# SUNGBEOMCHOI/Rubiks-Cube-Solver

Hardware: NVIDIA B200
Metric: cube transitions/sec (higher is better)
Workload: dtype u8

## Files before the change

rubiks_cube_solver_b200/csrc/build.py:

```python
import os
import subprocess
import sys

HERE = os.path.dirname(os.path.abspath(__file__))
PKG = os.path.dirname(HERE)
LIB = os.path.join(PKG, "libcube_b200.so")
SOURCES = ["scramble.cu", "prefix.cu", "walk.cu", "sched.cu", "expand.cu", "leaf.cu", "decode.cu", "adi.cu", "seeds.cu", "mcts.cu", "pipeline.cu", "envhost.cu", "peer.cu", "abi.cu"]
HEADERS = ["cube_common.cuh", "cube_threads.cuh", "cube_bulk.cuh", "cube_sched.cuh", "cube_tables.cuh", "cube_kernels.h", os.path.join("..", "..", "include", "cube_b200.h")]
NVCC_FLAGS = ["-O3", "-std=c++17", "-gencode", "arch=compute_100a,code=sm_100a", "-lineinfo",
              "-Xcompiler", "-fPIC", "-shared"]


def nvcc():
    for cand in (os.environ.get("NVCC"), "/usr/local/cuda/bin/nvcc", "nvcc"):
        if cand and (os.path.isabs(cand) and os.path.exists(cand) or not os.path.isabs(cand)):
            return cand
    return "nvcc"


def stale():
    if not os.path.exists(LIB):
        return True
    t = os.path.getmtime(LIB)
    return any(os.path.getmtime(os.path.join(HERE, f)) > t
               for f in SOURCES + HEADERS if os.path.exists(os.path.join(HERE, f)))


def build(force=False, verbose=False):
    from concurrent.futures import ThreadPoolExecutor
    srcs = [s for s in SOURCES if os.path.exists(os.path.join(HERE, s))]
    if not force and not stale():
        return LIB
    objdir = os.path.join(HERE, "build")
    os.makedirs(objdir, exist_ok=True)
    hdr_t = max(os.path.getmtime(os.path.join(HERE, h)) for h in HEADERS + ["build.py"] if os.path.exists(os.path.join(HERE, h)))
    compile_flags = [f for f in NVCC_FLAGS if f != "-shared"] + (["-Xptxas", "-v"] if verbose else [])

    def compile_one(src):
        obj = os.path.join(objdir, src[:-3] + ".o")
        if not force and os.path.exists(obj) and os.path.getmtime(obj) > max(hdr_t, os.path.getmtime(os.path.join(HERE, src))):
            return obj
        tmp_o = obj + ".tmp%d" % os.getpid()
        try:
            subprocess.check_call([nvcc()] + compile_flags + ["-c", "-o", tmp_o, src], cwd=HERE)
            os.replace(tmp_o, obj)
        finally:
            if os.path.exists(tmp_o):
                os.remove(tmp_o)
        return obj

    with ThreadPoolExecutor(max_workers=min(len(srcs), os.cpu_count() or 4)) as pool:
        objs = list(pool.map(compile_one, srcs))
    tmp = LIB + ".tmp%d" % os.getpid()
    try:
        subprocess.check_call([nvcc()] + NVCC_FLAGS + ["-o", tmp] + objs, cwd=HERE)
        os.replace(tmp, LIB)
    finally:
        if os.path.exists(tmp):
            os.remove(tmp)
    return LIB

# ... 4 lines not shown
```

rubiks_cube_solver_b200/csrc/cube_kernels.h:

```cpp
#pragma once
#include <cstdint>
#include <cuda_runtime.h>
#include "../../include/cube_b200.h"

namespace cube {

int launch_scramble(int size, const uint8_t* moves, long long n, int depth, uint8_t* states_out,
                    uint8_t* solved, float* reward, unsigned long long* counters, cudaStream_t stream,
                    const uint8_t* last = nullptr);

int launch_prefixes(int size, const uint8_t* moves, long long n, int depth, uint8_t* states_out, uint8_t* solved,
                    unsigned long long* counters, cudaStream_t stream);
int prefix_max_depth(int size);

int launch_walk(int size, const uint8_t* states_in, const uint8_t* moves, long long n, int depth,
                uint8_t* states_out, uint8_t* solved, float* reward, unsigned long long* counters,
                cudaStream_t stream);

int launch_solved(int size, const uint8_t* states, long long n, uint8_t* solved, float* reward,
                  unsigned long long* counters, cudaStream_t stream);

int launch_expand(int size, const uint8_t* states, long long n, uint8_t* children, void* child_onehot,
                  void* parent_onehot, int dtype, uint8_t* solved, float* reward,
                  unsigned long long* counters, cudaStream_t stream, int encoding = CUBE_ENCODING_REFERENCE);

int launch_expand_codes(int size, const uint8_t* states, long long n, uint8_t* children, uint8_t* child_codes,
                        uint8_t* parent_codes, void* parent_onehot, int dtype, uint8_t* solved, float* reward,
                        unsigned long long* counters, cudaStream_t stream, int encoding = CUBE_ENCODING_REFERENCE);

int launch_validate(int size, const uint8_t* actions, long long count, unsigned long long* counters,
                    cudaStream_t stream);

long long launch_leaf2(const uint8_t* states, long long n, uint8_t* children, void* parent_onehot, int dtype,
                       uint8_t* solved, float* reward, unsigned long long* counters, cudaStream_t stream, int* rc);

int launch_seeded_moves(int size, const uint32_t* seeds, long long n, int depth, uint8_t* moves,
                        unsigned long long* counters, cudaStream_t stream);

int launch_adi_targets(int size, const float* child_values, const uint8_t* child_solved, const float* parent_values,
                       const int* scramble_count, const double* weight, int table_len, long long n,
                       float* target_value, int* target_policy, double* error, cudaStream_t stream);

long long launch_leaf2_children(const uint8_t* states, long long n, uint8_t* children, void* child_onehot,
                                void* parent_onehot, int dtype, uint8_t* solved, float* reward,
                                unsigned long long* counters, cudaStream_t stream, int* rc);

int launch_mcts_traverse(int size, const cube_mcts_tree_t& t, float cpuct, int virtual_loss, cudaStream_t stream);
int launch_mcts_update(int size, const cube_mcts_tree_t& t, const uint8_t* leaf_key, const uint8_t* child_key_new,
                       const uint8_t* child_done_new, const float* value, const float* policy, float value_min,
                       int sim_index, int8_t* actions_out, int* n_actions, int* n_sims, int* n_active, cudaStream_t stream);

int launch_decode2(const void* onehot, int dtype, long long n, uint8_t* out, cudaStream_t stream);
int launch_decode3_exact(const void* onehot, int dtype, long long n, uint8_t* out, cudaStream_t stream);

size_t peer_buffer_bytes(int cap);
int launch_peer_allreduce_i64(int world, int rank, const uint64_t* peer_bufs, long long* values, int n, int cap,
                              unsigned epoch, cudaStream_t stream);

int sm_count();
int device_slot();
int persistent_ctas();

}
```

rubiks_cube_solver_b200/csrc/cube_sched.cuh:

```cuda
#pragma once
#include <cstdint>
#include <cuda_runtime.h>

namespace sched {

constexpr int kClaimChunk = 2;
constexpr int kRanges = 8;
constexpr int kTailDiv = 4;
constexpr int kSlots = 1024;
constexpr int kExhausted = 0x7fffff00;

struct Slot { unsigned next[kRanges][32]; unsigned ctas_done; unsigned tail_div; unsigned pad[30]; };

Slot* claim_slot();
int tail_div();

struct WarpTiles {
    Slot* slot;
    int n_tiles, total_warps, tail0;
    int next_static;
    int r, visited;
    int cur, end;
    int chunk;
    unsigned pending;

    __device__ __forceinline__ int lo(int range) const
    {
        return tail0 + (int)((long long)range * (n_tiles - tail0) / kRanges);
    }
    __device__ __forceinline__ void claim_ahead(int lane)
    {
        if (lane == 0) pending = atomicAdd(&slot->next[r][0], (unsigned)chunk);
    }

    __device__ __forceinline__ void init(Slot* s, int n, int warps_per_cta, int warp, int lane, int tail_div,
                                         int claim_chunk = kClaimChunk)
    {
        slot = s; n_tiles = n; total_warps = (int)gridDim.x * warps_per_cta; chunk = claim_chunk;
        const int gid = (int)blockIdx.x * warps_per_cta + warp;
        tail0 = tail_div > 0 ? n - n / tail_div : n;
        next_static = gid;
        r = gid % kRanges; visited = 0; cur = end = 0; pending = 0;
        if (next_static >= tail0) claim_ahead(lane);
    }

    __device__ __forceinline__ int pop(int lane)
    {
        if (next_static < tail0) {
            const int t = next_static;
            next_static += total_warps;
            if (next_static >= tail0) claim_ahead(lane);
            return t;
        }
        while (cur >= end) {
            if (visited >= kRanges) return kExhausted;
            const unsigned got = __shfl_sync(0xffffffffu, pending, 0);
            const int hi = lo(r + 1);
            const long long base = (long long)lo(r) + got;
            if (base < hi) {
                cur = (int)base;
                end = cur + chunk < hi ? cur + chunk : hi;
            } else {
                bool left = false;
                if (lane < kRanges) left = lo(lane) + (long long)__ldcg(&slot->next[lane][0]) < lo(lane + 1);
                const unsigned open = __ballot_sync(0xffffffffu, left) & ((1u << kRanges) - 1u);
                if (open == 0) { visited = kRanges; return kExhausted; }
                const unsigned rot = (open >> (r + 1)) | (open << (kRanges - r - 1));
                r = (r + 1 + (__ffs(rot & ((1u << kRanges) - 1u)) - 1)) % kRanges;
            }
            claim_ahead(lane);
        }
        return cur++;
    }
};

__device__ __forceinline__ void release(Slot* slot)
{
    if (threadIdx.x == 0) {
        __threadfence();
        if (atomicAdd(&slot->ctas_done, 1u) == gridDim.x - 1) {
            for (int i = 0; i < kRanges; ++i) slot->next[i][0] = 0;
            slot->ctas_done = 0;
            __threadfence();
        }
    }
}

}
```

rubiks_cube_solver_b200/csrc/sched.cu:

```cuda
#include <atomic>
#include <cstdlib>
#include "cube_sched.cuh"

namespace sched {

__device__ Slot g_slots[kSlots];

Slot* claim_slot()
{
    static std::atomic<unsigned> seq{0};
    static Slot* base[64] = {};
    int dev = 0;
    if (cudaGetDevice(&dev) != cudaSuccess || dev < 0 || dev >= 64) return nullptr;
    Slot* b = base[dev];
    if (!b) {
        void* p = nullptr;
        if (cudaGetSymbolAddress(&p, g_slots) != cudaSuccess) return nullptr;
        b = base[dev] = static_cast<Slot*>(p);
    }
    return b + (seq.fetch_add(1, std::memory_order_relaxed) % kSlots);
}

int tail_div()
{
    static int v = -1;
    if (v < 0) {
        const char* e = getenv("CUBE_TAIL_DIV");
        v = e ? atoi(e) : kTailDiv;
        if (v < 0) v = kTailDiv;
    }
    return v;
}

}
```

rubiks_cube_solver_b200/csrc/scramble.cu:

```cuda
#include <atomic>
#include <cstdlib>
#include <cstring>
#include <cuda.h>
#include <cuda_runtime.h>
#include "cube_bulk.cuh"
#include "cube_kernels.h"
#include "cube_sched.cuh"
#include "cube_threads.cuh"

namespace {

#ifndef CUBE_SCRAMBLE_MIN_BLOCKS
#define CUBE_SCRAMBLE_MIN_BLOCKS 6
#endif
constexpr int kTile = 256;
constexpr int kMaxStagedDepth = 160;

__host__ __device__ constexpr int round16(int x) { return (x + 15) & ~15; }

template <int SIZE>
struct ScrambleSmem {
    using G = CubeGeom<SIZE>;
    static constexpr int kTable = 0;
    static constexpr int kCornerLut = kTable + G::MW * CUBE_MOVE_ROWS * 4;
// ... 83 lines not shown
        }
    } else {
        const long long byte0 = base * G::S;
        const int nbytes = cnt * G::S;
        for (int i = tid; i < nbytes; i += kTile) out[byte0 + i] = s_out[i];
    }
    if (tid < cnt) {
        const bool row_ok = s_flags[tid] != 0;
        if (solved) solved[base + tid] = row_ok ? 1 : 0;
        if (reward) reward[base + tid] = row_ok ? 1.0f : -1.0f;
    }
    if (full && tid == 0) bulk::wait_read_all();
}


constexpr int kMaxPairDepth = 320;
constexpr int kPairTableBytes = CUBE_PAIR_ROWS * 256;
template <int SIZE, int NS> struct PairCfg;
template <> struct PairCfg<3, 2> { static constexpr int kMaxWarps = 24; };
template <> struct PairCfg<2, 2> { static constexpr int kMaxWarps = 32; };
template <> struct PairCfg<2, 4> { static constexpr int kMaxWarps = 20; };
constexpr int kMinWarpsFour = 16;

template <int SIZE, int NS>
struct PairSmem {
    using G = CubeGeom<SIZE>;
    static constexpr int kPairTile = 32 * NS;
    static constexpr int kTable = 0;
    static constexpr int kCornerLut = kPairTableBytes + 256;
    static constexpr int kEdgeLut = kCornerLut + 256;
    static constexpr int kPerWarp = (kEdgeLut + (SIZE == 3 ? 1536 : 256) + 1023) / 1024 * 1024;
    static constexpr int kOutBytes = kPairTile * G::S;
    __host__ __device__ static constexpr int round1k(int x) { return (x + 1023) & ~1023; }
    __host__ __device__ static constexpr int move_stride(int depth, bool swz = false)
    {
        return swz ? round1k(kPairTile * depth) : kPairTile * depth + 16;
    }
    __host__ __device__ static constexpr int moves_at(bool swz = false) { return swz ? round1k(16 + kOutBytes) : 16 + kOutBytes; }
    __host__ __device__ static constexpr int per_warp(int depth, bool swz = false)
    {
        return moves_at(swz) + 2 * move_stride(depth, swz);
    }
    __host__ __device__ static constexpr int bytes(int depth, int warps, bool priv = false)
    {
        return kPerWarp + warps * per_warp(depth, priv) < 66048 ? 66048 : kPerWarp + warps * per_warp(depth, priv);
    }
};

template <int SIZE, int DEPTH, int NS, int MODE>
__global__ void __launch_bounds__(PairCfg<SIZE, NS>::kMaxWarps * 32, 1)
scramble_pairs_kernel(const uint8_t* __restrict__ moves, int n_tiles, int depth_rt, uint8_t* __restrict__ out,
                      uint8_t* __restrict__ solved, float* __restrict__ reward, unsigned long long* __restrict__ counters,
                      sched::Slot* slot, int tail_div, const __grid_constant__ CUtensorMap move_map,
                      const uint8_t* __restrict__ last)
{
    using L = PairSmem<SIZE, NS>;
    constexpr int kPairTile = L::kPairTile;
    extern __shared__ __align__(128) uint8_t smem_raw[];
    const int depth = DEPTH > 0 ? DEPTH : depth_rt;
    constexpr bool kPriv = DEPTH < 0;
    constexpr uint32_t kAlign = kPriv ? 1024u : 256u;
    const int tid = threadIdx.x, lane = tid & 31, warp = tid >> 5;
    const uint32_t window = bulk::smem_addr(smem_raw);
    uint8_t* smem = smem_raw + ((kAlign - (window & (kAlign - 1u))) & (kAlign - 1u));
    uint8_t* s_ptbl = smem + L::kTable;
    const PairTableShared tbl{bulk::smem_addr(s_ptbl)};
    uint32_t* s_clut = reinterpret_cast<uint32_t*>(smem + L::kCornerLut);
    uint32_t* s_elut = reinterpret_cast<uint32_t*>(smem + L::kEdgeLut);
    uint8_t* mine = smem + L::kPerWarp + warp * L::per_warp(depth, kPriv);
    uint64_t* s_bar = reinterpret_cast<uint64_t*>(mine);
    uint8_t* s_out = mine + 16;
    uint8_t* s_moves = mine + L::moves_at(kPriv);
    const int mstride = L::move_stride(depth, kPriv);
    const uint32_t move_bytes = (uint32_t)(kPairTile * depth);
    auto stage = [&](int t, int b) {
        if (bulk::elect_one()) {
            bulk::mbar_expect_tx(&s_bar[b], move_bytes);
            if (!kPriv) bulk::load(s_moves + b * mstride, moves + (long long)t * move_bytes, move_bytes, &s_bar[b]);
            else bulk::load_tile_2d(s_moves + b * mstride, &move_map, 0, t * (kPairTile * depth >> 7), &s_bar[b]);
        }
    };

    asm volatile("griddepcontrol.launch_dependents;");
    pair_table_fill<SIZE>(s_ptbl, tid, blockDim.x);
    if (tid < 32) s_clut[tid] = (SIZE == 3) ? kCornerColour3[tid] : kCornerColour2[tid];
    if (SIZE == 3) for (int i = tid; i < 12 * 32; i += blockDim.x) s_elut[i] = kEdgeColourSlot3[i];
    if (lane == 0) { bulk::mbar_init(&s_bar[0], 1); bulk::mbar_init(&s_bar[1], 1); }
    if (lane == 0 && depth > 0) {
        const int total = (int)gridDim.x * (int)(blockDim.x >> 5);
#pragma unroll
        for (int k = 0; k < 2; ++k) {
            const int t = (int)blockIdx.x * (int)(blockDim.x >> 5) + warp + k * total;
            if (t < n_tiles) bulk::prefetch_l2(moves + (long long)t * move_bytes, move_bytes);
        }
    }
    __syncthreads();
    asm volatile("griddepcontrol.wait;" ::: "memory");

    sched::WarpTiles tiles;
    tiles.init(slot, n_tiles, (int)(blockDim.x >> 5), warp, lane, tail_div);
    int tile = tiles.pop(lane);
    if (tile < n_tiles) stage(tile, 0);
    int rows[NS];
#pragma unroll
    for (int k = 0; k < NS; ++k) rows[k] = (SIZE == 3) ? 64 * (k >> 1) + 2 * lane + (k & 1) : lane + 32 * k;
    const uint32_t lanereg = pair_lanereg<SIZE>(lane, tbl), roff = pair_roff2(lane);
    const ColourLutShared lut{bulk::smem_addr(s_clut), bulk::smem_addr(s_elut)};
    unsigned n_solved = 0;
    const bool has_last = MODE == 2 || (MODE == 0 && last != nullptr);
    const bool has_solved = MODE != 0 || solved != nullptr, has_reward = MODE != 0 || reward != nullptr;
    for (int it = 0; tile < n_tiles; ++it) {
        const int buf = it & 1;
        const int next = tiles.pop(lane);
        if (next < n_tiles) stage(next, buf ^ 1);
        uint32_t last_w[NS];
        if (has_last) {
            if (SIZE == 3) {
#pragma unroll
                for (int h = 0; h < NS; h += 2) {
                    const uint32_t v = *reinterpret_cast<const uint16_t*>(last + (long long)tile * kPairTile + 32 * h + 2 * lane);
                    last_w[h] = v & 0xffu; last_w[h + 1] = v >> 8;
                }
            } else {
#pragma unroll
                for (int k = 0; k < NS; ++k) last_w[k] = last[(long long)tile * kPairTile + 32 * k + lane];
            }
        }
        bulk::mbar_wait(&s_bar[buf], (uint32_t)(it >> 1) & 1u);

        CubieState st[NS];
#pragma unroll
        for (int k = 0; k < NS; ++k) cubie_init(st[k]);
        if constexpr (kPriv) scramble_pairs_run_swizzled<SIZE, NS>(st, s_moves + buf * mstride, lane, depth, tbl, lanereg, roff);
        else scramble_pairs_run<SIZE, (DEPTH > 0 ? DEPTH : 0), NS>(st, rows, depth, s_moves + buf * mstride, tbl, lanereg, roff);
        if (has_last) {
#pragma unroll
            for (int k = 0; k < NS; ++k) scramble_pairs_last<SIZE>(st[k], last_w[k], tbl, lanereg, roff);
        }
        if (bulk::elect_one()) bulk::wait_read_all();
        __syncwarp();
        bool ok[NS];
#pragma unroll
        for (int k = 0; k < NS; ++k) {
            ok[k] = scramble_pairs_finish<SIZE>(st[k], rows[k], lut, s_out);
            n_solved += ok[k] ? 1u : 0u;
        }

        bulk::fence_smem_writes();
        __syncwarp();
        if (bulk::elect_one()) {
            bulk::store(out + (long long)tile * L::kOutBytes, s_out, (uint32_t)L::kOutBytes);
            bulk::commit();
        }
        if (SIZE == 3) {
#pragma unroll
            for (int h = 0; h < NS; h += 2) {
                const long long r0 = (long long)tile * kPairTile + 32 * h + 2 * lane;
                if (has_solved) *reinterpret_cast<uint16_t*>(solved + r0) = (uint16_t)((ok[h] ? 1u : 0u) | (ok[h + 1] ? 0x100u : 0u));
                if (has_reward) *reinterpret_cast<float2*>(reward + r0) = make_float2(ok[h] ? 1.0f : -1.0f, ok[h + 1] ? 1.0f : -1.0f);
            }
        } else {
#pragma unroll
            for (int k = 0; k < NS; ++k) {
                if (has_solved) solved[(long long)tile * kPairTile + 32 * k + lane] = ok[k] ? 1 : 0;
                if (has_reward) reward[(long long)tile * kPairTile + 32 * k + lane] = ok[k] ? 1.0f : -1.0f;
            }
        }
        tile = next;
    }
    n_solved = __reduce_add_sync(0xffffffffu, n_solved);
    if (lane == 0 && n_solved && counters) atomicAdd(&counters[0], (unsigned long long)n_solved);
    if (blockIdx.x == 0 && tid == 0 && counters) atomicAdd(&counters[1], (unsigned long long)n_tiles * kPairTile);
    __syncwarp();
    if (bulk::elect_one()) bulk::wait_read_all();
    __syncthreads();
    sched::release(slot);
}

constexpr int kSliceDefault = 112;
__host__ __device__ constexpr int slice_stride(int slice) { return ((slice + 32) / 16) % 2 ? slice + 32 : slice + 48; }

template <int SIZE>
struct SlicedSmem {
    using G = CubeGeom<SIZE>;
    static constexpr int kOutBytes = 64 * G::S;
    static constexpr int kMovesAt = 16 + kOutBytes;
    __host__ __device__ static constexpr int per_warp(int slice) { return kMovesAt + 2 * 64 * slice_stride(slice); }
    static constexpr int kFixed = PairSmem<SIZE, 2>::kPerWarp;
    __host__ __device__ static constexpr int bytes(int warps, int slice) { return kFixed + warps * per_warp(slice); }
};

template <int SIZE>
__global__ void __launch_bounds__(8 * 32, 1)
scramble_sliced_kernel(const uint8_t* __restrict__ moves, int n_tiles, int depth, uint8_t* __restrict__ out,
                       uint8_t* __restrict__ solved, float* __restrict__ reward, unsigned long long* __restrict__ counters,
                       const uint8_t* __restrict__ last, int kSlice)
{
    using L = SlicedSmem<SIZE>;
    using P = PairSmem<SIZE, 2>;
    extern __shared__ __align__(128) uint8_t smem_raw[];
    const int tid = threadIdx.x, lane = tid & 31, warp = tid >> 5, warps = (int)(blockDim.x >> 5);
    const uint32_t window = bulk::smem_addr(smem_raw);
    uint8_t* smem = smem_raw + ((256u - (window & 255u)) & 255u);
    uint8_t* s_ptbl = smem + P::kTable;
    const PairTableShared tbl{bulk::smem_addr(s_ptbl)};
    uint32_t* s_clut = reinterpret_cast<uint32_t*>(smem + P::kCornerLut);
    uint32_t* s_elut = reinterpret_cast<uint32_t*>(smem + P::kEdgeLut);
    const int kSliceStride = slice_stride(kSlice);
    uint8_t* mine = smem + L::kFixed + warp * L::per_warp(kSlice);
    uint64_t* s_bar = reinterpret_cast<uint64_t*>(mine);
    uint8_t* s_out = mine + 16;
    uint8_t* s_moves = mine + L::kMovesAt;

    pair_table_fill<SIZE>(s_ptbl, tid, blockDim.x);
    if (tid < 32) s_clut[tid] = (SIZE == 3) ? kCornerColour3[tid] : kCornerColour2[tid];
    if (SIZE == 3) for (int i = tid; i < 12 * 32; i += blockDim.x) s_elut[i] = kEdgeColourSlot3[i];
    if (lane == 0) { bulk::mbar_init(&s_bar[0], 32); bulk::mbar_init(&s_bar[1], 32); }
    __syncthreads();

    const int n_slices = (depth + kSlice - 1) / kSlice;
// ... 162 lines not shown
        if (smem > configured_smem.load(std::memory_order_relaxed)) {
            cudaError_t e = cudaFuncSetAttribute(kern_full, cudaFuncAttributeMaxDynamicSharedMemorySize, smem);
            if (e == cudaSuccess) e = cudaFuncSetAttribute(kern_tail, cudaFuncAttributeMaxDynamicSharedMemorySize, smem);
            if (e != cudaSuccess) return (int)e;
            cudaFuncSetAttribute(kern_full, cudaFuncAttributePreferredSharedMemoryCarveout, cudaSharedmemCarveoutMaxShared);
            configured_smem.store(smem, std::memory_order_relaxed);
        }
        const long long full_tiles = n / kTile;
        if (full_tiles > 0)
            kern_full<<<(unsigned)full_tiles, kTile, smem, stream>>>(moves, n, 0, depth, out, solved, reward, counters, last);
        if (full_tiles < n_tiles)
            kern_tail<<<1, kTile, smem, stream>>>(moves, n, full_tiles, depth, out, solved, reward, counters, last);
    } else {
        auto kern = scramble_deep_kernel<SIZE>;
        int per_sm = 0;
        if (cudaOccupancyMaxActiveBlocksPerMultiprocessor(&per_sm, kern, kTile, smem) != cudaSuccess || per_sm < 1)
            per_sm = 1;
        long long grid = (long long)cube::sm_count() * per_sm;
        if (grid > n_tiles) grid = n_tiles;
        kern<<<(unsigned)grid, kTile, smem, stream>>>(moves, n, depth, out, solved, reward, counters, last);
    }
    return (int)cudaGetLastError();
}

constexpr int kSmemLimit = 227 * 1024;

using EncodeTiledFn = CUresult (*)(CUtensorMap*, CUtensorMapDataType, cuuint32_t, void*, const cuuint64_t*,
                                   const cuuint64_t*, const cuuint32_t*, const cuuint32_t*, CUtensorMapInterleave,
                                   CUtensorMapSwizzle, CUtensorMapL2promotion, CUtensorMapFloatOOBfill);

bool encode_move_map(CUtensorMap* map, const uint8_t* moves, long long n_tiles, int tile_rows)
{
    static const EncodeTiledFn encode = [] {
        void* p = nullptr;
        cudaDriverEntryPointQueryResult q = cudaDriverEntryPointSymbolNotFound;
        if (cudaGetDriverEntryPoint("cuTensorMapEncodeTiled", &p, cudaEnableDefault, &q) != cudaSuccess ||
            q != cudaDriverEntryPointSuccess)
            p = nullptr;
        (void)cudaGetLastError();
        return reinterpret_cast<EncodeTiledFn>(p);
    }();
    if (!encode) return false;
    const cuuint64_t dims[2] = {128, (cuuint64_t)(n_tiles * tile_rows)};
    const cuuint64_t strides[1] = {128};
    const cuuint32_t box[2] = {128, (cuuint32_t)tile_rows};
    const cuuint32_t elem[2] = {1, 1};
    return encode(map, CU_TENSOR_MAP_DATA_TYPE_UINT8, 2, const_cast<uint8_t*>(moves), dims, strides, box, elem,
                  CU_TENSOR_MAP_INTERLEAVE_NONE, CU_TENSOR_MAP_SWIZZLE_128B, CU_TENSOR_MAP_L2_PROMOTION_NONE,
                  CU_TENSOR_MAP_FLOAT_OOB_FILL_NONE) == CUDA_SUCCESS;
}

template <int SIZE, int NS>
long long launch_pairs(const uint8_t* moves, long long n, int depth, uint8_t* out, uint8_t* solved, float* reward,
                       unsigned long long* counters, cudaStream_t stream, int min_warps, const uint8_t* last)
{
    using L = PairSmem<SIZE, NS>;
    constexpr int kPairTile = L::kPairTile;
    if (n < kPairTile) return 0;
    static const bool swz_ok = !(getenv("CUBE_PAIR_SWIZZLE") && getenv("CUBE_PAIR_SWIZZLE")[0] == '0');
    static_assert(L::kPerWarp % 1024 == 0, "the per-warp areas of the swizzled variant start on 1 KB");
    long long n_tiles = n / kPairTile;
    if (n_tiles > 0x3fffffff) n_tiles = 0x3fffffff;
    const int tile_rows = kPairTile * depth / 128;
    constexpr bool kCanSwizzle = SIZE == 2 || NS == 2;
    bool priv = kCanSwizzle && swz_ok && depth % (SIZE == 3 ? 8 : 16) == 0 && n_tiles * tile_rows < 0x7fffffffLL;
    auto warps_for = [&](bool p) {
        int w = (kSmemLimit - (p ? 1024 : 256) - L::kPerWarp) / L::per_warp(depth, p);
        if (w > PairCfg<SIZE, NS>::kMaxWarps) w = PairCfg<SIZE, NS>::kMaxWarps;
        return w & ~3;
    };
    if (warps_for(priv) < min_warps) return 0;
    alignas(64) CUtensorMap move_map;
    memset(&move_map, 0, sizeof(move_map));
    if (priv && !encode_move_map(&move_map, moves, n_tiles, tile_rows)) priv = false;
    const int slack = priv ? 1024 : 256;
    const int warps = warps_for(priv);
    if (warps < min_warps) return 0;
    const int smem = L::bytes(depth, warps, priv) + slack;
    constexpr int kM2 = SIZE == 3 ? 2 : 0;
    const int mode = (solved && reward) ? (last ? kM2 : 1) : 0;
    const int variant = depth == 30 ? 1 : depth == 20 ? 2 : priv ? 3 : 0;
    using Kern = decltype(&scramble_pairs_kernel<SIZE, 0, NS, 0>);
    constexpr int kSwz = kCanSwizzle ? -1 : 0;
    static const Kern kerns[3][4] = {
        {scramble_pairs_kernel<SIZE, 0, NS, 0>, scramble_pairs_kernel<SIZE, 30, NS, 0>, scramble_pairs_kernel<SIZE, 20, NS, 0>, scramble_pairs_kernel<SIZE, kSwz, NS, 0>},
        {scramble_pairs_kernel<SIZE, 0, NS, 1>, scramble_pairs_kernel<SIZE, 30, NS, 1>, scramble_pairs_kernel<SIZE, 20, NS, 1>, scramble_pairs_kernel<SIZE, kSwz, NS, 1>},
        {scramble_pairs_kernel<SIZE, 0, NS, kM2>, scramble_pairs_kernel<SIZE, 30, NS, kM2>, scramble_pairs_kernel<SIZE, 20, NS, kM2>, scramble_pairs_kernel<SIZE, kSwz, NS, kM2>}};
    const Kern kern = kerns[mode][variant];
    static std::atomic<int> configured_smem[64][12];
    std::atomic<int>& cfg = configured_smem[cube::device_slot()][variant + 4 * mode];
    if (smem > cfg.load(std::memory_order_relaxed)) {
        cudaError_t e = cudaFuncSetAttribute(kern, cudaFuncAttributeMaxDynamicSharedMemorySize, smem);
        if (e != cudaSuccess) return -(long long)e;
        cfg.store(smem, std::memory_order_relaxed);
    }
    long long grid = (n_tiles + warps - 1) / warps;
    if (grid > cube::persistent_ctas()) grid = cube::persistent_ctas();
    sched::Slot* slot = sched::claim_slot();
    if (!slot) return -(long long)cudaErrorUnknown;
    cudaLaunchConfig_t cfg_l = {};
    cfg_l.gridDim = dim3((unsigned)grid);
    cfg_l.blockDim = dim3((unsigned)(warps * 32));
    cfg_l.dynamicSmemBytes = (size_t)smem;
    cfg_l.stream = stream;
    cudaLaunchAttribute attr[1];
    attr[0].id = cudaLaunchAttributeProgrammaticStreamSerialization;
    attr[0].val.programmaticStreamSerializationAllowed = 1;
    static const bool pdl = !(getenv("CUBE_PDL") && getenv("CUBE_PDL")[0] == '0');
    cfg_l.attrs = attr;
    cfg_l.numAttrs = pdl ? 1 : 0;
    cudaError_t e = cudaLaunchKernelEx(&cfg_l, kern, moves, (int)n_tiles, depth, out, solved, reward, counters, slot,
                                       sched::tail_div(), move_map, last);
    if (e == cudaSuccess) e = cudaGetLastError();
    if (e != cudaSuccess) return -(long long)e;
    return n_tiles * kPairTile;
}

template <int SIZE>
int launch_one(const uint8_t* moves, long long n, int depth, uint8_t* out, uint8_t* solved, float* reward,
               unsigned long long* counters, cudaStream_t stream, const uint8_t* last)
{
    using G = CubeGeom<SIZE>;
    long long done = 0;
    static const char* const force = getenv("CUBE_SCRAMBLE_CLASSIC");
    static const bool four_ok = !(getenv("CUBE_PAIR_FOUR") && getenv("CUBE_PAIR_FOUR")[0] == '0');
    const bool aligned = ((reinterpret_cast<uintptr_t>(solved) & 1u) | (reinterpret_cast<uintptr_t>(reward) & 7u) |
                          (reinterpret_cast<uintptr_t>(last) & 1u)) == 0;
    if (depth >= 1 && depth <= kMaxPairDepth && aligned && !(force && force[0] == '1')) {
        if (SIZE == 2 && four_ok)
            done = launch_pairs<2, 4>(moves, n, depth, out, solved, reward, counters, stream, kMinWarpsFour, last);
        if (done == 0) done = launch_pairs<SIZE, 2>(moves, n, depth, out, solved, reward, counters, stream, 4, last);
        if (done < 0) return (int)-done;
    }
    static const bool sliced_ok = !(getenv("CUBE_PAIR_SLICED") && getenv("CUBE_PAIR_SLICED")[0] == '0');
    if (depth > kMaxPairDepth && aligned && sliced_ok && !(force && force[0] == '1')) {
        done = launch_sliced<SIZE>(moves, n, depth, out, solved, reward, counters, stream, last);
        if (done < 0) return (int)-done;
    }
    if (done == n) return 0;
    return launch_classic<SIZE>(moves + done * depth, n - done, depth, out + done * G::S, solved ? solved + done : nullptr,
                                reward ? reward + done : nullptr, counters, stream, last ? last + done : nullptr);
}

}

namespace cube {

int launch_scramble(int size, const uint8_t* moves, long long n, int depth, uint8_t* states_out,
                    uint8_t* solved, float* reward, unsigned long long* counters, cudaStream_t stream, const uint8_t* last)
{
    if (n == 0) return 0;
    if (size == 3) return launch_one<3>(moves, n, depth, states_out, solved, reward, counters, stream, last);
    return launch_one<2>(moves, n, depth, states_out, solved, reward, counters, stream, last);
}

}
```

rubiks_cube_solver_b200/csrc/seeds.cu:

```cuda
#include <cuda_runtime.h>
#include "cube_kernels.h"
#include "../../include/cube_b200.h"

namespace {

template <int K>
__device__ __forceinline__ uint32_t shr(uint32_t x)
{
    return __umulhi(x, 1u << (32 - K));
}

__device__ __forceinline__ uint32_t mt_next_seed_word(uint32_t prev, uint32_t j)
{
    return 1812433253u * (prev ^ shr<30>(prev)) + j;
}

constexpr int kSeedThreads = 128;

struct SeedIndex { uint32_t v[400]; };
constexpr SeedIndex make_seed_index()
{
    SeedIndex t{};
    for (int j = 0; j < 400; ++j) t.v[j] = (uint32_t)j;
    return t;
// ... 10 lines not shown
    const long long i = base + tid;
    if (i < n) {
        const uint32_t seed = seeds[i];
        uint32_t z = seed;
#pragma unroll
        for (int j = 1; j <= 397; ++j) z = mt_next_seed_word(z, kSeedIndex.v[j]);
        uint32_t x = seed, xn = mt_next_seed_word(seed, 1), idx = 0;
        uint32_t p = (uint32_t)__cvta_generic_to_shared(s_rows) + (uint32_t)(tid * depth);
        const uint32_t end = p + (uint32_t)depth;
        while (p < end && idx < 227) {
            const uint32_t y = (x & 0x80000000u) | (xn & 0x7fffffffu);
            uint32_t v = z ^ shr<1>(y) ^ ((y & 1u) ? 0x9908b0dfu : 0u);
            v ^= shr<11>(v);
            v ^= (v << 7) & 0x9d2c5680u;
            v ^= (v << 15) & 0xefc60000u;
            v ^= shr<18>(v);
            ++idx;
            x = xn;
            xn = mt_next_seed_word(xn, idx + 1);
            z = mt_next_seed_word(z, idx + 397);
            const uint32_t val = v & mask;
            if (val <= max_value) {
                asm volatile("st.shared.u8 [%0], %1;" ::"r"(p), "r"(val) : "memory");
                ++p;
            }
        }
        if (p < end) {
            for (; p < end; ++p) asm volatile("st.shared.u8 [%0], %1;" ::"r"(p), "r"((uint32_t)CUBE_NOOP) : "memory");
            if (counters) atomicAdd(&counters[3], 1ull);
        }
    }
    __syncthreads();
    const long long rows = (n - base) < (long long)kSeedThreads ? (n - base) : (long long)kSeedThreads;
    const int nbytes = (int)rows * depth;
    uint8_t* dst = moves + base * depth;
    const int nvec = nbytes >> 4;
    for (int v = tid; v < nvec; v += kSeedThreads)
        reinterpret_cast<int4*>(dst)[v] = reinterpret_cast<const int4*>(s_rows)[v];
    for (int k = (nvec << 4) + tid; k < nbytes; k += kSeedThreads) dst[k] = s_rows[k];
}

}

namespace cube {

int launch_seeded_moves(int size, const uint32_t* seeds, long long n, int depth, uint8_t* moves,
                        unsigned long long* counters, cudaStream_t stream)
{
    if (n == 0 || depth == 0) return 0;
    const uint32_t max_value = size == 3 ? 11u : 5u;
    uint32_t mask = max_value;
    mask |= mask >> 1; mask |= mask >> 2; mask |= mask >> 4; mask |= mask >> 8; mask |= mask >> 16;
    const long long blocks = (n + kSeedThreads - 1) / kSeedThreads;
    seeded_moves_kernel<<<(unsigned)blocks, kSeedThreads, (size_t)kSeedThreads * depth, stream>>>(seeds, n, depth, max_value,
                                                                                                   mask, moves, counters);
    return (int)cudaGetLastError();
}

}
```

rubiks_cube_solver_b200/csrc/walk.cu:

```cuda
#include <atomic>
#include <cstdlib>
#include <cuda_runtime.h>
#include "cube_bulk.cuh"
#include "cube_kernels.h"
#include "cube_sched.cuh"
#include "cube_threads.cuh"

namespace {

constexpr int kTile = 256;

__host__ __device__ constexpr int round16(int x) { return (x + 15) & ~15; }

template <int SIZE, bool FULL>
__global__ void __launch_bounds__(kTile, 6)
walk_tile_kernel(const uint8_t* in, const uint8_t* __restrict__ moves, long long n, long long tile0, int depth,
                 uint8_t* out, uint8_t* __restrict__ solved, float* __restrict__ reward,
                 unsigned long long* __restrict__ counters)
{
    using G = CubeGeom<SIZE>;
    __shared__ __align__(128) uint8_t s_rows[round16(kTile * G::S)];
    __shared__ uint32_t s_cyc[G::NCYC * CUBE_MOVE_ROWS];
    __shared__ uint8_t s_flags[kTile];
    __shared__ __align__(8) uint64_t s_bar;
// ... 44 lines not shown
        } else {
            const long long byte0 = base * G::S;
            for (int i = tid; i < cnt * G::S; i += kTile) out[byte0 + i] = s_rows[i];
        }
    }
    if (tid < cnt) {
        const bool row_ok = s_flags[tid] != 0;
        if (solved) solved[base + tid] = row_ok ? 1 : 0;
        if (reward) reward[base + tid] = row_ok ? 1.0f : -1.0f;
    }
    if (FULL && out && tid == 0) bulk::wait_read_all();
}


constexpr int kRowsPerTile = 64;
constexpr int kMaxWalkWarps = 24;
constexpr int kMaxPrivateDepth = 64;

template <int SIZE>
struct WalkSmem {
    using G = CubeGeom<SIZE>;
    static constexpr int kEntries = 0;
    static constexpr int kPerWarp = 2 * G::NCYC * CUBE_MOVE_ROWS * 8;
    static constexpr int kTileBytes = kRowsPerTile * G::S;
    static constexpr int kScratch = 32 * WalkImage<SIZE>::W * 4;
    __host__ __device__ static constexpr int move_stride(int depth) { return kRowsPerTile * depth + 16; }
    __host__ __device__ static constexpr int per_warp(int depth)
    {
        return 16 + 2 * (kTileBytes + 16) + kScratch + 2 * move_stride(depth);
    }
    __host__ __device__ static constexpr int bytes(int depth, int warps) { return kPerWarp + warps * per_warp(depth); }
};

template <int SIZE>
__global__ void __launch_bounds__(kMaxWalkWarps * 32, 1)
walk_private_kernel(const uint8_t* in, const uint8_t* __restrict__ moves, int n_tiles, int depth, uint8_t* out,
                    uint8_t* __restrict__ solved, float* __restrict__ reward, unsigned long long* __restrict__ counters,
                    sched::Slot* slot, int tail_div)
{
    using G = CubeGeom<SIZE>;
    using L = WalkSmem<SIZE>;
    constexpr int W = WalkImage<SIZE>::W;
    extern __shared__ __align__(128) uint8_t smem[];
    const int tid = threadIdx.x, lane = tid & 31, warp = tid >> 5;
    uint32_t* s_ent = reinterpret_cast<uint32_t*>(smem + L::kEntries);
    uint8_t* mine = smem + L::kPerWarp + warp * L::per_warp(depth);
    uint64_t* s_bar = reinterpret_cast<uint64_t*>(mine);
    uint8_t* s_tile = mine + 16;
    uint8_t* s_scratch = s_tile + 2 * (L::kTileBytes + 16);
    uint8_t* s_moves = s_scratch + L::kScratch;
    const int mstride = L::move_stride(depth);
    const uint32_t move_bytes = (uint32_t)(kRowsPerTile * depth);

    asm volatile("griddepcontrol.launch_dependents;");
    for (int i = tid; i < 2 * G::NCYC * CUBE_MOVE_ROWS; i += blockDim.x) {
        const int shift = (i >= G::NCYC * CUBE_MOVE_ROWS) ? 2 : 0;
        const int cm = i - (shift ? G::NCYC * CUBE_MOVE_ROWS : 0);
        walk_cycle_entry((SIZE == 3) ? kCycles3[cm] : kCycles2[cm], shift, s_ent + 2 * i);
    }
    if (lane == 0) { bulk::mbar_init(&s_bar[0], 1); bulk::mbar_init(&s_bar[1], 1); }
    __syncthreads();
    asm volatile("griddepcontrol.wait;" ::: "memory");

    sched::WarpTiles tiles;
    tiles.init(slot, n_tiles, (int)(blockDim.x >> 5), warp, lane, tail_div);
    int tile = tiles.pop(lane);
    if (lane == 0 && tile < n_tiles) {
        bulk::mbar_expect_tx(&s_bar[0], (uint32_t)L::kTileBytes + move_bytes);
        bulk::load(s_tile, in + (long long)tile * L::kTileBytes, (uint32_t)L::kTileBytes, &s_bar[0]);
        bulk::load(s_moves, moves + (long long)tile * move_bytes, move_bytes, &s_bar[0]);
    }
    uint8_t* lane_base = s_scratch + 4 * lane;
    unsigned n_solved = 0;

    for (int it = 0; tile < n_tiles; ++it) {
        const int buf = it & 1;
        const int next = tiles.pop(lane);
        if (lane == 0) {
            bulk::wait_read_all();
            if (next < n_tiles) {
                bulk::mbar_expect_tx(&s_bar[buf ^ 1], (uint32_t)L::kTileBytes + move_bytes);
                bulk::load(s_tile + (buf ^ 1) * (L::kTileBytes + 16), in + (long long)next * L::kTileBytes,
                           (uint32_t)L::kTileBytes, &s_bar[buf ^ 1]);
                bulk::load(s_moves + (buf ^ 1) * mstride, moves + (long long)next * move_bytes, move_bytes, &s_bar[buf ^ 1]);
            }
        }
        bulk::mbar_wait(&s_bar[buf], (uint32_t)(it >> 1) & 1u);
        uint8_t* tile_p = s_tile + buf * (L::kTileBytes + 16);
        const uint8_t* moves_p = s_moves + buf * mstride;

        unsigned mask[2];
#pragma unroll
        for (int pass = 0; pass < 2; ++pass) {
            const int row = (SIZE == 3) ? 2 * lane + pass : lane + 32 * pass;
            constexpr int kShiftOdd = (SIZE == 3) ? 2 : 0;
            const int shift = pass ? kShiftOdd : 0;
            uint32_t* img_p = reinterpret_cast<uint32_t*>(tile_p + G::S * row - shift);
            uint32_t w[W];
            if (SIZE == 3) {
#pragma unroll
                for (int j = 0; j < W; ++j) w[j] = img_p[j];
            } else {
                const uint2* q = reinterpret_cast<const uint2*>(img_p);
#pragma unroll
                for (int j = 0; j < 3; ++j) { const uint2 v = q[j]; w[2 * j] = v.x; w[2 * j + 1] = v.y; }
            }
            const uint8_t* mrow = moves_p + row * depth;
            if (SIZE == 3) {
#pragma unroll
                for (int j = 0; j < W; ++j) reinterpret_cast<uint32_t*>(lane_base)[32 * j] = w[j];
                const uint32_t* ent = s_ent + (shift ? 2 * G::NCYC * CUBE_MOVE_ROWS : 0);
                for (int k = 0; k < depth; ++k) walk_turn_private<SIZE>(lane_base, ent, (uint32_t)mrow[k] & 0xfu);
#pragma unroll
                for (int j = 0; j < W; ++j) w[j] = reinterpret_cast<const uint32_t*>(lane_base)[32 * j];
            } else {
// ... 91 lines not shown
    if (depth >= 1 && depth <= kMaxPrivateDepth && out && n >= kRowsPerTile && aligned && !(force && force[0] == '1')) {
        int warps = (227 * 1024 - L::kPerWarp) / L::per_warp(depth);
        if (warps > kMaxWalkWarps) warps = kMaxWalkWarps;
        warps &= ~3;
        if (warps >= 8) {
            long long n_tiles = n / kRowsPerTile;
            if (n_tiles > 0x3fffffff) n_tiles = 0x3fffffff;
            const int smem = L::bytes(depth, warps);
            auto kern = walk_private_kernel<SIZE>;
            static std::atomic<int> configured_dev[64];
            std::atomic<int>& configured_smem = configured_dev[cube::device_slot()];
            if (smem > configured_smem.load(std::memory_order_relaxed)) {
                const cudaError_t e = cudaFuncSetAttribute(kern, cudaFuncAttributeMaxDynamicSharedMemorySize, smem);
                if (e != cudaSuccess) return (int)e;
                configured_smem.store(smem, std::memory_order_relaxed);
            }
            long long grid = (n_tiles + warps - 1) / warps;
            if (grid > cube::persistent_ctas()) grid = cube::persistent_ctas();
            sched::Slot* slot = sched::claim_slot();
            if (!slot) return (int)cudaErrorUnknown;
            cudaLaunchConfig_t cfg_l = {};
            cfg_l.gridDim = dim3((unsigned)grid);
            cfg_l.blockDim = dim3((unsigned)(warps * 32));
            cfg_l.dynamicSmemBytes = (size_t)smem;
            cfg_l.stream = stream;
            cudaLaunchAttribute attr[1];
            attr[0].id = cudaLaunchAttributeProgrammaticStreamSerialization;
            attr[0].val.programmaticStreamSerializationAllowed = 1;
            static const bool pdl = !(getenv("CUBE_PDL") && getenv("CUBE_PDL")[0] == '0');
            cfg_l.attrs = attr;
            cfg_l.numAttrs = pdl ? 1 : 0;
            cudaError_t e = cudaLaunchKernelEx(&cfg_l, kern, in, moves, (int)n_tiles, depth, out, solved, reward, counters, slot,
                                               sched::tail_div());
            if (e == cudaSuccess) e = cudaGetLastError();
            if (e != cudaSuccess) return (int)e;
            done = n_tiles * kRowsPerTile;
        }
    }
    if (done == n) return 0;
    return launch_classic<SIZE>(in + done * G::S, moves ? moves + done * depth : nullptr, n - done, depth,
                                out ? out + done * G::S : nullptr, solved ? solved + done : nullptr,
                                reward ? reward + done : nullptr, counters, stream);
}

}

namespace cube {

int launch_walk(int size, const uint8_t* states_in, const uint8_t* moves, long long n, int depth,
                uint8_t* states_out, uint8_t* solved, float* reward, unsigned long long* counters,
                cudaStream_t stream)
{
    if (n == 0) return 0;
    if (size == 3) return launch_tiles<3>(states_in, moves, n, depth, states_out, solved, reward, counters, stream);
    return launch_tiles<2>(states_in, moves, n, depth, states_out, solved, reward, counters, stream);
}

int launch_solved(int size, const uint8_t* states, long long n, uint8_t* solved, float* reward,
                  unsigned long long* counters, cudaStream_t stream)
{
    if (n == 0) return 0;
    if (size == 3) return launch_tiles<3>(states, nullptr, n, 0, nullptr, solved, reward, counters, stream);
    return launch_tiles<2>(states, nullptr, n, 0, nullptr, solved, reward, counters, stream);
}

int launch_validate(int size, const uint8_t* actions, long long count, unsigned long long* counters,
                    cudaStream_t stream)
{
    if (count == 0) return 0;
    long long blocks = (count / 16 + 255) / 256;
    const long long cap = (long long)sm_count() * 8;
    if (blocks > cap) blocks = cap;
    if (blocks < 1) blocks = 1;
    validate_kernel<<<(unsigned)blocks, 256, 0, stream>>>(actions, count, size == 3 ? 12u : 6u, counters);
    return (int)cudaGetLastError();
}

}
```

Measured before the change: 1426 billion.

## Let scramble kernel process its first tile before griddepcontrol.wait when inputs are unaffected

Adds a host-side per-stream record of the buffers each launch writes. With it, the scramble launcher can tell when its move/last inputs do not overlap the previous kernel's outputs. When that holds, each warp stages and walks its first statically assigned tile before griddepcontrol.wait and only stores results after the wait, overlapping the first tile's compute with the previous kernel's tail. launch_dependents is moved after the wait in scramble and walk kernels, and every launch now takes a global mutex plus map lookups on the host, which adds some per-launch overhead.

```diff
diff --git a/rubiks_cube_solver_b200/csrc/build.py b/rubiks_cube_solver_b200/csrc/build.py
--- a/rubiks_cube_solver_b200/csrc/build.py
+++ b/rubiks_cube_solver_b200/csrc/build.py
@@ -6,7 +6,7 @@
 PKG = os.path.dirname(HERE)
 LIB = os.path.join(PKG, "libcube_b200.so")
 SOURCES = ["scramble.cu", "prefix.cu", "walk.cu", "sched.cu", "expand.cu", "leaf.cu", "decode.cu", "adi.cu", "seeds.cu", "mcts.cu", "pipeline.cu", "envhost.cu", "peer.cu", "abi.cu"]
-HEADERS = ["cube_common.cuh", "cube_threads.cuh", "cube_bulk.cuh", "cube_sched.cuh", "cube_tables.cuh", "cube_kernels.h", os.path.join("..", "..", "include", "cube_b200.h")]
+HEADERS = ["cube_common.cuh", "cube_threads.cuh", "cube_bulk.cuh", "cube_sched.cuh", "cube_pdl.cuh", "cube_tables.cuh", "cube_kernels.h", os.path.join("..", "..", "include", "cube_b200.h")]
 NVCC_FLAGS = ["-O3", "-std=c++17", "-gencode", "arch=compute_100a,code=sm_100a", "-lineinfo",
               "-Xcompiler", "-fPIC", "-shared"]
 
diff --git a/rubiks_cube_solver_b200/csrc/cube_kernels.h b/rubiks_cube_solver_b200/csrc/cube_kernels.h
--- a/rubiks_cube_solver_b200/csrc/cube_kernels.h
+++ b/rubiks_cube_solver_b200/csrc/cube_kernels.h
@@ -2,6 +2,7 @@
 #include <cstdint>
 #include <cuda_runtime.h>
 #include "../../include/cube_b200.h"
+#include "cube_pdl.cuh"
 
 namespace cube {
 
@@ -57,6 +58,23 @@
 int launch_peer_allreduce_i64(int world, int rank, const uint64_t* peer_bufs, long long* values, int n, int cap,
                               unsigned epoch, cudaStream_t stream);
 
+class StreamWrites {
+public:
+    explicit StreamWrites(cudaStream_t stream);
+    ~StreamWrites();
+    StreamWrites(const StreamWrites&) = delete;
+    StreamWrites& operator=(const StreamWrites&) = delete;
+    bool may_read_early(const pdl::Span* reads, int k) const;
+    void note(const pdl::Span* writes, int k);
+
+private:
+    cudaStream_t stream_;
+    pdl::Record* rec_;
+    bool capturing_;
+    const cudaGraphNode_t* deps_;
+    size_t n_deps_;
+};
+
 int sm_count();
 int device_slot();
 int persistent_ctas();
diff --git a/rubiks_cube_solver_b200/csrc/cube_pdl.cuh b/rubiks_cube_solver_b200/csrc/cube_pdl.cuh
--- /dev/null
+++ b/rubiks_cube_solver_b200/csrc/cube_pdl.cuh
@@ -0,0 +1,51 @@
+#pragma once
+#include <cstddef>
+#include <cstdint>
+
+namespace pdl {
+
+struct Span { uintptr_t lo, hi; };
+
+inline Span span(const void* p, size_t bytes)
+{
+    const uintptr_t a = reinterpret_cast<uintptr_t>(p);
+    return {a, p ? a + bytes : a};
+}
+
+inline bool overlaps(Span a, Span b) { return a.lo < a.hi && b.lo < b.hi && a.lo < b.hi && b.lo < a.hi; }
+
+constexpr int kMaxSpans = 4;
+
+struct Record {
+    Span w[kMaxSpans] = {};
+    int n = 0;
+    const void* node = nullptr;
+
+    void note(const Span* s, int k, const void* graph_node = nullptr)
+    {
+        n = 0;
+        node = graph_node;
+        for (int i = 0; i < k; ++i) {
+            if (s[i].lo >= s[i].hi) continue;
+            if (n < kMaxSpans) { w[n++] = s[i]; continue; }
+            Span& h = w[kMaxSpans - 1];
+            if (s[i].lo < h.lo) h.lo = s[i].lo;
+            if (s[i].hi > h.hi) h.hi = s[i].hi;
+        }
+    }
+
+    bool may_read_early(const Span* r, int k, bool capturing = false, const void* const* deps = nullptr,
+                        size_t n_deps = 0) const
+    {
+        if (capturing) {
+            if (n_deps == 0) return true;
+            if (n_deps != 1 || node == nullptr || deps[0] != node) return false;
+        }
+        for (int i = 0; i < k; ++i)
+            for (int j = 0; j < n; ++j)
+                if (overlaps(r[i], w[j])) return false;
+        return true;
+    }
+};
+
+}
diff --git a/rubiks_cube_solver_b200/csrc/cube_sched.cuh b/rubiks_cube_solver_b200/csrc/cube_sched.cuh
--- a/rubiks_cube_solver_b200/csrc/cube_sched.cuh
+++ b/rubiks_cube_solver_b200/csrc/cube_sched.cuh
@@ -28,6 +28,7 @@
     {
         return tail0 + (int)((long long)range * (n_tiles - tail0) / kRanges);
     }
+    __device__ __forceinline__ static int tail_start(int n, int tail_div) { return tail_div > 0 ? n - n / tail_div : n; }
     __device__ __forceinline__ void claim_ahead(int lane)
     {
         if (lane == 0) pending = atomicAdd(&slot->next[r][0], (unsigned)chunk);
@@ -38,7 +39,7 @@
     {
         slot = s; n_tiles = n; total_warps = (int)gridDim.x * warps_per_cta; chunk = claim_chunk;
         const int gid = (int)blockIdx.x * warps_per_cta + warp;
-        tail0 = tail_div > 0 ? n - n / tail_div : n;
+        tail0 = tail_start(n, tail_div);
         next_static = gid;
         r = gid % kRanges; visited = 0; cur = end = 0; pending = 0;
         if (next_static >= tail0) claim_ahead(lane);
diff --git a/rubiks_cube_solver_b200/csrc/sched.cu b/rubiks_cube_solver_b200/csrc/sched.cu
--- a/rubiks_cube_solver_b200/csrc/sched.cu
+++ b/rubiks_cube_solver_b200/csrc/sched.cu
@@ -1,5 +1,10 @@
 #include <atomic>
 #include <cstdlib>
+#include <map>
+#include <mutex>
+#include <thread>
+#include <tuple>
+#include "cube_kernels.h"
 #include "cube_sched.cuh"
 
 namespace sched {
@@ -33,3 +38,58 @@
 }
 
 }
+
+namespace cube {
+namespace {
+
+using StreamKey = std::tuple<int, uintptr_t, std::thread::id, unsigned long long>;
+std::mutex g_mu;
+std::map<StreamKey, pdl::Record> g_records;
+constexpr size_t kMaxRecords = 1 << 14;
+
+}
+
+StreamWrites::StreamWrites(cudaStream_t stream) : stream_(stream), capturing_(false), deps_(nullptr), n_deps_(0)
+{
+    g_mu.lock();
+    cudaStreamCaptureStatus cs = cudaStreamCaptureStatusNone;
+    unsigned long long capture = 0;
+    if (cudaStreamGetCaptureInfo(stream, &cs, &capture, nullptr, &deps_, &n_deps_) != cudaSuccess) {
+        (void)cudaGetLastError();
+        cs = cudaStreamCaptureStatusNone;
+    }
+    capturing_ = cs == cudaStreamCaptureStatusActive;
+    if (!capturing_) capture = 0, deps_ = nullptr, n_deps_ = 0;
+    uintptr_t h = reinterpret_cast<uintptr_t>(stream);
+    if (h == reinterpret_cast<uintptr_t>(cudaStreamLegacy)) h = 0;
+    const std::thread::id thread = h == reinterpret_cast<uintptr_t>(cudaStreamPerThread) ? std::this_thread::get_id()
+                                                                                       : std::thread::id();
+    if (g_records.size() >= kMaxRecords) {
+        for (auto it = g_records.begin(); it != g_records.end();)
+            it = std::get<3>(it->first) ? g_records.erase(it) : std::next(it);
+    }
+    rec_ = &g_records[StreamKey(device_slot(), h, thread, capture)];
+}
+
+StreamWrites::~StreamWrites() { g_mu.unlock(); }
+
+bool StreamWrites::may_read_early(const pdl::Span* reads, int k) const
+{
+    static const bool on = !(getenv("CUBE_PDL_EARLY") && getenv("CUBE_PDL_EARLY")[0] == '0');
+    return on && rec_->may_read_early(reads, k, capturing_, reinterpret_cast<const void* const*>(deps_), n_deps_);
+}
+
+void StreamWrites::note(const pdl::Span* writes, int k)
+{
+    const void* node = nullptr;
+    if (capturing_) {
+        cudaStreamCaptureStatus cs = cudaStreamCaptureStatusNone;
+        const cudaGraphNode_t* deps = nullptr;
+        size_t n = 0;
+        if (cudaStreamGetCaptureInfo(stream_, &cs, nullptr, nullptr, &deps, &n) == cudaSuccess && n == 1) node = deps[0];
+        else (void)cudaGetLastError();
+    }
+    rec_->note(writes, k, node);
+}
+
+}
diff --git a/rubiks_cube_solver_b200/csrc/scramble.cu b/rubiks_cube_solver_b200/csrc/scramble.cu
--- a/rubiks_cube_solver_b200/csrc/scramble.cu
+++ b/rubiks_cube_solver_b200/csrc/scramble.cu
@@ -159,7 +159,7 @@
 scramble_pairs_kernel(const uint8_t* __restrict__ moves, int n_tiles, int depth_rt, uint8_t* __restrict__ out,
                       uint8_t* __restrict__ solved, float* __restrict__ reward, unsigned long long* __restrict__ counters,
                       sched::Slot* slot, int tail_div, const __grid_constant__ CUtensorMap move_map,
-                      const uint8_t* __restrict__ last)
+                      const uint8_t* __restrict__ last, int early)
 {
     using L = PairSmem<SIZE, NS>;
     constexpr int kPairTile = L::kPairTile;
@@ -188,26 +188,22 @@
         }
     };
 
-    asm volatile("griddepcontrol.launch_dependents;");
     pair_table_fill<SIZE>(s_ptbl, tid, blockDim.x);
     if (tid < 32) s_clut[tid] = (SIZE == 3) ? kCornerColour3[tid] : kCornerColour2[tid];
     if (SIZE == 3) for (int i = tid; i < 12 * 32; i += blockDim.x) s_elut[i] = kEdgeColourSlot3[i];
     if (lane == 0) { bulk::mbar_init(&s_bar[0], 1); bulk::mbar_init(&s_bar[1], 1); }
-    if (lane == 0 && depth > 0) {
-        const int total = (int)gridDim.x * (int)(blockDim.x >> 5);
+    const int warps_per_cta = (int)(blockDim.x >> 5), total = (int)gridDim.x * warps_per_cta;
+    const int gid = (int)blockIdx.x * warps_per_cta + warp, tail0 = sched::WarpTiles::tail_start(n_tiles, tail_div);
+    const bool pre = early && gid < tail0;
+    if (!pre && lane == 0) {
 #pragma unroll
         for (int k = 0; k < 2; ++k) {
-            const int t = (int)blockIdx.x * (int)(blockDim.x >> 5) + warp + k * total;
+            const int t = gid + k * total;
             if (t < n_tiles) bulk::prefetch_l2(moves + (long long)t * move_bytes, move_bytes);
         }
     }
     __syncthreads();
-    asm volatile("griddepcontrol.wait;" ::: "memory");
-
-    sched::WarpTiles tiles;
-    tiles.init(slot, n_tiles, (int)(blockDim.x >> 5), warp, lane, tail_div);
-    int tile = tiles.pop(lane);
-    if (tile < n_tiles) stage(tile, 0);
+
     int rows[NS];
 #pragma unroll
     for (int k = 0; k < NS; ++k) rows[k] = (SIZE == 3) ? 64 * (k >> 1) + 2 * lane + (k & 1) : lane + 32 * k;
@@ -216,10 +212,7 @@
     unsigned n_solved = 0;
     const bool has_last = MODE == 2 || (MODE == 0 && last != nullptr);
     const bool has_solved = MODE != 0 || solved != nullptr, has_reward = MODE != 0 || reward != nullptr;
-    for (int it = 0; tile < n_tiles; ++it) {
-        const int buf = it & 1;
-        const int next = tiles.pop(lane);
-        if (next < n_tiles) stage(next, buf ^ 1);
+    auto walk_tile = [&](int tile, int buf, int it, bool (&ok)[NS]) {
         uint32_t last_w[NS];
         if (has_last) {
             if (SIZE == 3) {
@@ -246,13 +239,13 @@
         }
         if (bulk::elect_one()) bulk::wait_read_all();
         __syncwarp();
-        bool ok[NS];
 #pragma unroll
         for (int k = 0; k < NS; ++k) {
             ok[k] = scramble_pairs_finish<SIZE>(st[k], rows[k], lut, s_out);
             n_solved += ok[k] ? 1u : 0u;
         }
-
+    };
+    auto send_tile = [&](int tile, const bool (&ok)[NS]) {
         bulk::fence_smem_writes();
         __syncwarp();
         if (bulk::elect_one()) {
@@ -273,6 +266,43 @@
                 if (has_reward) reward[(long long)tile * kPairTile + 32 * k + lane] = ok[k] ? 1.0f : -1.0f;
             }
         }
+    };
+
+    sched::WarpTiles tiles;
+    int tile, it = 0;
+    if (pre) {
+        tile = gid;
+        stage(tile, 0);
+        int next = gid + total < tail0 ? gid + total : -1;
+        if (next >= 0) stage(next, 1);
+        bool ok[NS];
+        walk_tile(tile, 0, 0, ok);
+        asm volatile("griddepcontrol.wait;" ::: "memory");
+        asm volatile("griddepcontrol.launch_dependents;");
+        tiles.init(slot, n_tiles, warps_per_cta, warp, lane, tail_div);
+        tiles.pop(lane);
+        const int got = tiles.pop(lane);
+        if (got != next) {
+            next = got;
+            if (next < n_tiles) stage(next, 1);
+        }
+        send_tile(tile, ok);
+        tile = next;
+        it = 1;
+    } else {
+        asm volatile("griddepcontrol.wait;" ::: "memory");
+        asm volatile("griddepcontrol.launch_dependents;");
+        tiles.init(slot, n_tiles, warps_per_cta, warp, lane, tail_div);
+        tile = tiles.pop(lane);
+        if (tile < n_tiles) stage(tile, 0);
+    }
+    for (; tile < n_tiles; ++it) {
+        const int buf = it & 1;
+        const int next = tiles.pop(lane);
+        if (next < n_tiles) stage(next, buf ^ 1);
+        bool ok[NS];
+        walk_tile(tile, buf, it, ok);
+        send_tile(tile, ok);
         tile = next;
     }
     n_solved = __reduce_add_sync(0xffffffffu, n_solved);
@@ -541,7 +571,7 @@
 
 template <int SIZE, int NS>
 long long launch_pairs(const uint8_t* moves, long long n, int depth, uint8_t* out, uint8_t* solved, float* reward,
-                       unsigned long long* counters, cudaStream_t stream, int min_warps, const uint8_t* last)
+                       unsigned long long* counters, cudaStream_t stream, int min_warps, const uint8_t* last, bool early)
 {
     using L = PairSmem<SIZE, NS>;
     constexpr int kPairTile = L::kPairTile;
@@ -599,7 +629,7 @@
     cfg_l.attrs = attr;
     cfg_l.numAttrs = pdl ? 1 : 0;
     cudaError_t e = cudaLaunchKernelEx(&cfg_l, kern, moves, (int)n_tiles, depth, out, solved, reward, counters, slot,
-                                       sched::tail_div(), move_map, last);
+                                       sched::tail_div(), move_map, last, (pdl && early) ? 1 : 0);
     if (e == cudaSuccess) e = cudaGetLastError();
     if (e != cudaSuccess) return -(long long)e;
     return n_tiles * kPairTile;
@@ -607,7 +637,7 @@
 
 template <int SIZE>
 int launch_one(const uint8_t* moves, long long n, int depth, uint8_t* out, uint8_t* solved, float* reward,
-               unsigned long long* counters, cudaStream_t stream, const uint8_t* last)
+               unsigned long long* counters, cudaStream_t stream, const uint8_t* last, bool early)
 {
     using G = CubeGeom<SIZE>;
     long long done = 0;
@@ -617,8 +647,8 @@
                           (reinterpret_cast<uintptr_t>(last) & 1u)) == 0;
     if (depth >= 1 && depth <= kMaxPairDepth && aligned && !(force && force[0] == '1')) {
         if (SIZE == 2 && four_ok)
-            done = launch_pairs<2, 4>(moves, n, depth, out, solved, reward, counters, stream, kMinWarpsFour, last);
-        if (done == 0) done = launch_pairs<SIZE, 2>(moves, n, depth, out, solved, reward, counters, stream, 4, last);
+            done = launch_pairs<2, 4>(moves, n, depth, out, solved, reward, counters, stream, kMinWarpsFour, last, early);
+        if (done == 0) done = launch_pairs<SIZE, 2>(moves, n, depth, out, solved, reward, counters, stream, 4, last, early);
         if (done < 0) return (int)-done;
     }
     static const bool sliced_ok = !(getenv("CUBE_PAIR_SLICED") && getenv("CUBE_PAIR_SLICED")[0] == '0');
@@ -639,8 +669,16 @@
                     uint8_t* solved, float* reward, unsigned long long* counters, cudaStream_t stream, const uint8_t* last)
 {
     if (n == 0) return 0;
-    if (size == 3) return launch_one<3>(moves, n, depth, states_out, solved, reward, counters, stream, last);
-    return launch_one<2>(moves, n, depth, states_out, solved, reward, counters, stream, last);
-}
-
-}
+    const long long S = size == 3 ? 54 : 24;
+    StreamWrites rec(stream);
+    const pdl::Span reads[2] = {pdl::span(moves, (size_t)(n * depth)), pdl::span(last, (size_t)n)};
+    const bool early = rec.may_read_early(reads, 2);
+    const int rc = size == 3 ? launch_one<3>(moves, n, depth, states_out, solved, reward, counters, stream, last, early)
+                             : launch_one<2>(moves, n, depth, states_out, solved, reward, counters, stream, last, early);
+    const pdl::Span writes[4] = {pdl::span(states_out, (size_t)(n * S)), pdl::span(solved, (size_t)n),
+                                 pdl::span(reward, (size_t)n * sizeof(float)), pdl::span(counters, 4 * sizeof(*counters))};
+    rec.note(writes, 4);
+    return rc;
+}
+
+}
diff --git a/rubiks_cube_solver_b200/csrc/seeds.cu b/rubiks_cube_solver_b200/csrc/seeds.cu
--- a/rubiks_cube_solver_b200/csrc/seeds.cu
+++ b/rubiks_cube_solver_b200/csrc/seeds.cu
@@ -86,8 +86,11 @@
     uint32_t mask = max_value;
     mask |= mask >> 1; mask |= mask >> 2; mask |= mask >> 4; mask |= mask >> 8; mask |= mask >> 16;
     const long long blocks = (n + kSeedThreads - 1) / kSeedThreads;
+    StreamWrites rec(stream);
     seeded_moves_kernel<<<(unsigned)blocks, kSeedThreads, (size_t)kSeedThreads * depth, stream>>>(seeds, n, depth, max_value,
                                                                                                    mask, moves, counters);
+    const pdl::Span writes[2] = {pdl::span(moves, (size_t)(n * depth)), pdl::span(counters, 4 * sizeof(*counters))};
+    rec.note(writes, 2);
     return (int)cudaGetLastError();
 }
 
diff --git a/rubiks_cube_solver_b200/csrc/walk.cu b/rubiks_cube_solver_b200/csrc/walk.cu
--- a/rubiks_cube_solver_b200/csrc/walk.cu
+++ b/rubiks_cube_solver_b200/csrc/walk.cu
@@ -120,7 +120,6 @@
     const int mstride = L::move_stride(depth);
     const uint32_t move_bytes = (uint32_t)(kRowsPerTile * depth);
 
-    asm volatile("griddepcontrol.launch_dependents;");
     for (int i = tid; i < 2 * G::NCYC * CUBE_MOVE_ROWS; i += blockDim.x) {
         const int shift = (i >= G::NCYC * CUBE_MOVE_ROWS) ? 2 : 0;
         const int cm = i - (shift ? G::NCYC * CUBE_MOVE_ROWS : 0);
@@ -129,6 +128,7 @@
     if (lane == 0) { bulk::mbar_init(&s_bar[0], 1); bulk::mbar_init(&s_bar[1], 1); }
     __syncthreads();
     asm volatile("griddepcontrol.wait;" ::: "memory");
+    asm volatile("griddepcontrol.launch_dependents;");
 
     sched::WarpTiles tiles;
     tiles.init(slot, n_tiles, (int)(blockDim.x >> 5), warp, lane, tail_div);
@@ -326,16 +326,26 @@
                 cudaStream_t stream)
 {
     if (n == 0) return 0;
-    if (size == 3) return launch_tiles<3>(states_in, moves, n, depth, states_out, solved, reward, counters, stream);
-    return launch_tiles<2>(states_in, moves, n, depth, states_out, solved, reward, counters, stream);
+    StreamWrites rec(stream);
+    const int rc = size == 3 ? launch_tiles<3>(states_in, moves, n, depth, states_out, solved, reward, counters, stream)
+                             : launch_tiles<2>(states_in, moves, n, depth, states_out, solved, reward, counters, stream);
+    const pdl::Span writes[4] = {pdl::span(states_out, (size_t)n * (size == 3 ? 54 : 24)), pdl::span(solved, (size_t)n),
+                                 pdl::span(reward, (size_t)n * sizeof(float)), pdl::span(counters, 4 * sizeof(*counters))};
+    rec.note(writes, 4);
+    return rc;
 }
 
 int launch_solved(int size, const uint8_t* states, long long n, uint8_t* solved, float* reward,
                   unsigned long long* counters, cudaStream_t stream)
 {
     if (n == 0) return 0;
-    if (size == 3) return launch_tiles<3>(states, nullptr, n, 0, nullptr, solved, reward, counters, stream);
-    return launch_tiles<2>(states, nullptr, n, 0, nullptr, solved, reward, counters, stream);
+    StreamWrites rec(stream);
+    const int rc = size == 3 ? launch_tiles<3>(states, nullptr, n, 0, nullptr, solved, reward, counters, stream)
+                             : launch_tiles<2>(states, nullptr, n, 0, nullptr, solved, reward, counters, stream);
+    const pdl::Span writes[3] = {pdl::span(solved, (size_t)n), pdl::span(reward, (size_t)n * sizeof(float)),
+                                 pdl::span(counters, 4 * sizeof(*counters))};
+    rec.note(writes, 3);
+    return rc;
 }
 
 int launch_validate(int size, const uint8_t* actions, long long count, unsigned long long* counters,
```

Measured after the change: 1431 billion, median of 6. Within noise of the previous version (+0.3%).
